# GStreamer/gst-plugins-bad

Measured on AMD Instinct MI355X. Metric: bayer2rgb Mpix/s @4K (device-resident batch), higher is better.
Workload: dtype u8

## Files before the change

gst-plugins-bad_amd/csrc/mibayer_internal.h:

```cpp
#ifndef MIBAYER_INTERNAL_H
#define MIBAYER_INTERNAL_H

#include <hip/hip_runtime.h>
#include <stddef.h>
#include <stdint.h>

namespace mibayer {

constexpr int kNumXcd = 8;

struct FastDiv {
  uint32_t d;
  uint32_t mul;
  uint32_t sh1, sh2;
};

inline FastDiv make_fastdiv (uint32_t d)
{
  FastDiv f;
  f.d = d ? d : 1;
  uint32_t l = 0;
  while (l < 32 && (1ull << l) < f.d)
    l++;
  f.mul = (uint32_t) ((((1ull << l) - f.d) << 32) / f.d + 1);
// ... 94 lines not shown
  uint32_t sel[4];
  int swap_rows;
  int nlist;
  const uint8_t *src_list[kMaxList];
  uint8_t *dst_list[kMaxList];
};

__device__ __forceinline__ const uint8_t *frame_src (const KParams &p, uint32_t frame)
{
  return p.nlist ? p.src_list[frame] : p.src + frame * p.src_frame_bytes;
}

__device__ __forceinline__ uint8_t *frame_dst (const KParams &p, uint32_t frame)
{
  return p.nlist ? p.dst_list[frame] : p.dst + frame * p.dst_frame_bytes;
}

struct Variant {
  const char *name;
  int tile_w;
  int tile_h;
  int threads;
  int band;
  int persistent;
  void (*fast) (KParams);
  void (*generic) (KParams);
  void (*aligned64) (KParams);
  void (*aligned128) (KParams);
};

int variant_count ();
const Variant &variant (int id);
int resolve_variant (int id, int width);
bool known_width_plan (int width, int *variant, int *band);
int frame_class_variant (int width, int height, int slots);
int plain_store_twin (int id);
int hybrid_store_twin (int id);
int production_shape_of (int id);

struct R2BParams {
  const uint8_t *src;
  uint8_t *dst;
  unsigned long long src_frame_bytes;
  unsigned long long dst_frame_bytes;
  int width;
  int height;
  int src_stride;
  int dst_stride;
  int out_dwords;
  long long total_rows;
  int band;
  int start_sleep;
  TileMap map;
  FastDiv div_height;
  uint32_t sel_lo[2];
  uint32_t sel_hi[2];
  int flat_k, flat_px, flat_ld, rows;
  FastDiv div_out_dwords;
  uint32_t item0, item_end;
  int nlist;
  FastDiv div_blocks_per_frame;
  const uint8_t *src_list[kMaxList];
  uint8_t *dst_list[kMaxList];
};
hipError_t launch_rgb2bayer (const R2BParams &p, bool vec16, hipStream_t stream,
    long long row0 = 0, long long nrows = -1);
hipError_t launch_rgb2bayer_list (const R2BParams &p, bool vec16, bool dst8, hipStream_t stream);

constexpr int kStripRows = 16;
struct DeepParams {
  const uint8_t *src;
  uint8_t *dst;
  unsigned long long src_frame_bytes;
  unsigned long long dst_frame_bytes;
  int width;
  int height;
  int src_stride;
  int dst_stride;
  int dn_last;
  int swap_rows;
  uint32_t in_sel;
  uint32_t mask2;
  int out_shift;
  uint32_t sel[4];
  uint32_t sel16[2][2];
  int green_odd;
  int red_odd;
  int vmax;
  uint32_t sel_cgd[2][2];
  int px3;
  int planar;
  int groups;
  FastDiv div_tiles_x;
  FastDiv div_chunks;
  uint32_t chunk0;
  uint32_t nwaves;
  int nlist;
  const uint8_t *src_list[kMaxList];
  uint8_t *dst_list[kMaxList];
};
struct ColourStage {
  int has_tone;
  int black[3];
  int m_hi[9], m_lo[9];
  uint32_t tone[257];
};
struct ColourParams {
  DeepParams d;
  int mhc;
  int in8, out16;
  ColourStage s;
};
struct StripKind { bool mhc, in8, out16; };
hipError_t launch_strip (const DeepParams &p, StripKind kind, const ColourStage *stage, int nframes, hipStream_t stream,
    long long chunk0 = 0, long long nchunks = -1);

constexpr int kHalfLanePixels = 4;
constexpr int kHalfWavePixels = 64 * kHalfLanePixels;
constexpr int kHalfGroupPixels = 4 * kHalfWavePixels;
constexpr int kHalfRows = 4;
struct HalfParams {
  DeepParams d;
  int in8, out16;
  int colour;
  ColourStage s;
};
hipError_t launch_half (const DeepParams &p, bool in8, bool out16, const ColourStage *stage, int nframes,
    hipStream_t stream);

constexpr int kStatsSegRows = 64;
constexpr int kStatsMaxZones = 64;
struct StatsParams {
  const uint8_t *src;
  unsigned long long src_frame_bytes;
  unsigned long long *stats;
  int width, height, src_stride;
  int in8;
  uint32_t in_sel;
  uint32_t mask2;
  uint32_t lo, hi;
  int zones_x, zones_y;
  int ch;
  FastDiv div_cw;
  int row_dwords;
  int segs;
  FastDiv div_strips;
};
hipError_t launch_stats (const StatsParams &p, int nframes, hipStream_t stream);

constexpr int kHistReps = 8;
constexpr int kHistAhead = 8;
constexpr int kHistMaxRows = 256;
constexpr int kHistMinRows = 16;
constexpr int kHistSpread = 512;
struct HistParams {
  const uint8_t *src;
  unsigned long long src_frame_bytes;
  uint32_t *hist;
  int src_stride;
  int in8;
  uint32_t in_sel;
  uint32_t mask2;
  int shift;
  int x0, x1, y0, y1;
  int g0, g1;
  int seg_rows;
  FastDiv div_strips;
};
hipError_t launch_hist (const HistParams &p, int nframes, hipStream_t stream);

struct FocusParams {
  const uint8_t *src;
  unsigned long long src_frame_bytes;
  unsigned long long *focus;
  int width, height, src_stride;
  int in8;
  uint32_t in_sel;
  uint32_t mask2;
  uint32_t thr;
  int zones_x, zones_y;
  int ch;
  FastDiv div_cw;
  int row_dwords;
  int segs;
  FastDiv div_strips;
};
hipError_t launch_focus (const FocusParams &p, int nframes, hipStream_t stream);

constexpr int kShadeAhead = 8;
constexpr int kShadeMaxRows = 64;
constexpr int kShadeMinRows = 16;
constexpr int kShadeSpread = 1024;
constexpr int kShadeMaxNodes = 129;
struct ShadeParams {
  const uint8_t *src;
  uint8_t *dst;
  unsigned long long src_frame_bytes, dst_frame_bytes;
  const uint16_t *table;
  int width, height, src_stride, dst_stride;
  int in8;
  uint32_t in_sel;
  uint32_t mask2;
  int vmax;
  int kx, ky;
  int nx, ny;
  int black[4];
  int y0, y1;
  int row_dwords;
  int seg_rows;
  FastDiv div_strips;
};
hipError_t launch_shade (const ShadeParams &p, int nframes, hipStream_t stream);

constexpr int kDpcMaxRows = 64;
constexpr int kDpcMinRows = 16;
constexpr int kDpcSpread = 1024;
struct DpcParams {
  const uint8_t *src;
  uint8_t *dst;
  unsigned long long src_frame_bytes, dst_frame_bytes;
  const uint32_t *list;
  int list_lo, list_hi;
  int width, height, src_stride, dst_stride;
  int in8;
  uint32_t in_sel;
  uint32_t mask2;
  int hot, cold;
  int y0, y1;
  int row_dwords;
  int seg_rows;
  FastDiv div_strips;
};
hipError_t launch_dpc (const DpcParams &p, int nframes, hipStream_t stream);

constexpr int kNrMaxRows = 64;
constexpr int kNrMinRows = 16;
constexpr int kNrSpread = 1024;
struct NrParams {
  const uint8_t *src;
  uint8_t *dst;
  unsigned long long src_frame_bytes, dst_frame_bytes;
  int width, height, src_stride, dst_stride;
  int in8;
  uint32_t in_sel;
  uint32_t mask2;
  int shift;
  int y0, y1;
  int lut[16][2];
  uint32_t rcp[26];
// ... 15 lines not shown
```

gst-plugins-bad_amd/csrc/mibayer_kernels.hip:

```cpp
#include "mibayer_internal.h"

#include <stdlib.h>
#include <type_traits>

namespace mibayer {

typedef uint32_t u32x4 __attribute__ ((ext_vector_type (4)));
typedef uint32_t u32x2 __attribute__ ((ext_vector_type (2)));
typedef uint32_t u32x4_a4 __attribute__ ((ext_vector_type (4), aligned (4)));
typedef uint32_t u32x2_a4 __attribute__ ((ext_vector_type (2), aligned (4)));
typedef uint32_t u32x3_a4 __attribute__ ((ext_vector_type (3), aligned (4)));


template <bool INTRIN>
__device__ __forceinline__ uint32_t avg4 (uint32_t a, uint32_t b)
{
  if constexpr (INTRIN) {
    return __builtin_amdgcn_lerp (a, b, 0x01010101u);
  } else {
    return (a | b) - (((a ^ b) >> 1) & 0x7f7f7f7fu);
  }
}

template <bool INTRIN>
// ... 1413 lines not shown
  }
  uint32_t q[4];
  q[0] = from_lane_below (e, hi);
  q[1] = lo;
  q[2] = hi;
  q[3] = from_lane_above (e, lo);
  if (first)
    q[0] = bsel (kLowHalves, q[2], q[1]);
  if (lastmode == 1)
    q[3] = bsel (kLowHalves, q[2], q[1]);
  if (partial)
    q[2] = bsel (kLowHalves, q[1], q[0]);
  int s[8];
#pragma unroll
  for (int i = 0; i < 4; i++) {
    s[2 * i] = (int) (q[i] & 0xffffu);
    s[2 * i + 1] = (int) (q[i] >> 16);
  }
  MhcRow r;
#pragma unroll
  for (int k = 0; k < 4; k++) {
    r.c[k] = s[k + 2];
    r.h1[k] = s[k + 1] + s[k + 3];
    r.h2[k] = s[k] + s[k + 4];
  }
  return r;
}

template <bool GREEN>
__device__ __forceinline__ void mhc_pixel (const DeepParams &p, const MhcRow &m2, const MhcRow &m1, const MhcRow &z,
    const MhcRow &p1, const MhcRow &p2, int k, int &C, int &G, int &D)
{
  const int c = z.c[k];
  const int h1 = z.h1[k], h2 = z.h2[k];
  const int v1 = m1.c[k] + p1.c[k];
  const int v2 = m2.c[k] + p2.c[k];
  const int d = m1.h1[k] + p1.h1[k];
  int f1, f2;
  if constexpr (GREEN) {
    G = c;
    f1 = 10 * c + 8 * h1 - 2 * (h2 + d) + v2;
    f2 = 10 * c + 8 * v1 - 2 * (v2 + d) + h2;
  } else {
    C = c;
    f1 = 8 * c + 4 * (h1 + v1) - 2 * (h2 + v2);
    f2 = 12 * c + 4 * d - 3 * (h2 + v2);
  }
  f1 = min (max ((f1 + 8) >> 4, 0), p.vmax);
  f2 = min (max ((f2 + 8) >> 4, 0), p.vmax);
  if constexpr (GREEN)
    C = f1;
  else
    G = f1;
  D = f2;
}

__device__ __forceinline__ int reflect_row (int r, int height)
{
  r = r < 0 ? -r : r;
  return r > height + 1 ? height - 1 : r >= height ? 2 * height - 2 - r : r;
}

template <bool OUT16>
__device__ __forceinline__ void emit_cgd (const uint32_t (&x)[4], const uint32_t (&y)[4], uint32_t s0, uint32_t s1,
    u32x4 &v0, u32x4 &v1)
{
  if constexpr (OUT16) {
    v0.x = __builtin_amdgcn_perm (x[0], y[0], s0);
    v0.y = __builtin_amdgcn_perm (x[0], y[0], s1);
    v0.z = __builtin_amdgcn_perm (x[1], y[1], s0);
    v0.w = __builtin_amdgcn_perm (x[1], y[1], s1);
    v1.x = __builtin_amdgcn_perm (x[2], y[2], s0);
    v1.y = __builtin_amdgcn_perm (x[2], y[2], s1);
    v1.z = __builtin_amdgcn_perm (x[3], y[3], s0);
    v1.w = __builtin_amdgcn_perm (x[3], y[3], s1);
  } else {
    v0.x = __builtin_amdgcn_perm (x[0], y[0], s0);
    v0.y = __builtin_amdgcn_perm (x[1], y[1], s0);
    v0.z = __builtin_amdgcn_perm (x[2], y[2], s0);
    v0.w = __builtin_amdgcn_perm (x[3], y[3], s0);
  }
}

template <bool IN8, bool OUT16>
__global__ void __launch_bounds__ (256)
bayer2rgb_mhc_kernel (DeepParams p)
{
  const uint32_t wave = (uint32_t) __builtin_amdgcn_readfirstlane ((int) (blockIdx.x * 4u + (threadIdx.x >> 6)));
  if (wave >= p.nwaves)
    return;
  const int lane = (int) (threadIdx.x & 63u);
  const uint32_t crow = fastdiv (wave, p.div_tiles_x);
  const uint32_t tx = wave - crow * p.div_tiles_x.d;
  const uint32_t chunk = p.chunk0 + crow;
  const uint32_t frame = fastdiv (chunk, p.div_chunks);
  const int y0 = (int) (chunk - frame * p.div_chunks.d) * kStripRows;
  const int y1 = y0 + kStripRows < p.height ? y0 + kStripRows : p.height;
  const uint8_t *src = p.nlist
      ? kernarg_table_entry<const uint8_t *> (offsetof (DeepParams, src_list), frame) : p.src + frame * p.src_frame_bytes;
  uint8_t *dst = p.nlist
      ? kernarg_table_entry<uint8_t *> (offsetof (DeepParams, dst_list), frame) : p.dst + frame * p.dst_frame_bytes;
  const int g = (int) tx * 64 + lane;
  const bool first = g == 0;
  const int lastmode = g == p.groups - 1 ? ((p.width & 3) ? 2 : 1) : 0;
  const bool store = g < p.groups;
  const bool full = 4 * g + 4 <= p.width;

  DeepRaw raw[kStripRows + 4];
#pragma unroll
  for (int i = 0; i < kStripRows + 4; i++)
    raw[i] = deep_load<IN8> (p, src, reflect_row (y0 - 2 + i, p.height), g, lane);
  MhcRow w0 = mhc_row<IN8> (p, raw[0], lane, first, lastmode);
  MhcRow w1 = mhc_row<IN8> (p, raw[1], lane, first, lastmode);
  MhcRow w2 = mhc_row<IN8> (p, raw[2], lane, first, lastmode);
  MhcRow w3 = mhc_row<IN8> (p, raw[3], lane, first, lastmode);
#pragma unroll
  for (int k = 0; k < kStripRows; k++) {
    const int j = y0 + k;
    if (j >= y1)
      break;
    const MhcRow w4 = mhc_row<IN8> (p, raw[k + 4], lane, first, lastmode);
    int C[4], G[4], D[4];
    if (((j & 1) ^ p.green_odd) == 0) {
      mhc_pixel<true> (p, w0, w1, w2, w3, w4, 0, C[0], G[0], D[0]);
      mhc_pixel<false> (p, w0, w1, w2, w3, w4, 1, C[1], G[1], D[1]);
      mhc_pixel<true> (p, w0, w1, w2, w3, w4, 2, C[2], G[2], D[2]);
      mhc_pixel<false> (p, w0, w1, w2, w3, w4, 3, C[3], G[3], D[3]);
    } else {
      mhc_pixel<false> (p, w0, w1, w2, w3, w4, 0, C[0], G[0], D[0]);
      mhc_pixel<true> (p, w0, w1, w2, w3, w4, 1, C[1], G[1], D[1]);
      mhc_pixel<false> (p, w0, w1, w2, w3, w4, 2, C[2], G[2], D[2]);
      mhc_pixel<true> (p, w0, w1, w2, w3, w4, 3, C[3], G[3], D[3]);
    }
    const int rk = (j & 1) ^ p.red_odd;
    const int s = p.out_shift;
    uint32_t x[4], y[4];
#pragma unroll
    for (int i = 0; i < 4; i++) {
      if constexpr (OUT16) {
        x[i] = ((uint32_t) C[i] << s) | ((uint32_t) G[i] << (16 + s));
        y[i] = (uint32_t) D[i] << s;
      } else {
        x[i] = ((uint32_t) C[i] >> s) | (((uint32_t) G[i] >> s) << 16);
        y[i] = (uint32_t) D[i] >> s;
      }
    }
    uint8_t *out = dst + (size_t) j * (size_t) p.dst_stride;
    if constexpr (OUT16) {
      const uint32_t s0 = p.sel_cgd[rk][0], s1 = p.sel_cgd[rk][1];
      u32x4 v0, v1;
      emit_cgd<true> (x, y, s0, s1, v0, v1);
      store_strip16 (p, out, g, lane, v0, v1);
    } else if (const int planes = planar_of (p)) {
      store_planes8 (p, planes, out, g, store, full, rk ? 2 : 0, rk ? 0 : 2, gather_byte<0> (x), gather_byte<2> (x),
          gather_byte<0> (y));
    } else {
      const uint32_t s0 = p.sel_cgd[rk][0];
      u32x4 v, unused;
      emit_cgd<false> (x, y, s0, s0, v, unused);
      store_strip8 (out, g, store, full, p.px3 != 0, v);
    }
    w0 = w1;
    w1 = w2;
    w2 = w3;
    w3 = w4;
  }
}


constexpr int kColourAhead = 4;

__device__ __forceinline__ DeepRaw colour_load (const ColourParams &cp, const uint8_t *src, int r, int g, int lane)
{
  const DeepParams &p = cp.d;
  if (cp.mhc) {
    r = reflect_row (r, p.height);
  } else {
    r = r < 0 ? -r : r;
    r = r == p.height ? p.dn_last : r > p.height ? p.height - 1 : r;
  }
  if (cp.in8)
    return deep_load<true> (p, src, r, g, lane);
  return deep_load<false> (p, src, r, g, lane);
}

__device__ __forceinline__ MhcRow colour_row (const ColourParams &cp, const DeepRaw &raw, int lane, bool first,
    int lastmode)
{
  MhcRow r;
  if (cp.in8)
    r = mhc_row<true> (cp.d, raw, lane, first, lastmode);
  else
    r = mhc_row<false> (cp.d, raw, lane, first, lastmode);
  if (!cp.mhc) {
// ... 549 lines not shown
        const uint32_t m = __builtin_amdgcn_perm (d, d, p.in_sel) & p.mask2;
        v[0] = m & 0xffffu;
        v[1] = m >> 16;
        v[2] = v[3] = 0;
      }
#pragma unroll
      for (int k = 0; k < 4; k++) {
        const uint32_t wk = k < 2 ? w : w & w23;
        const bool in = v[k] - p.lo <= p.hi - p.lo;
        sum[rp][k >> 1][k & 1] += in ? v[k] * wk : 0u;
        cnt[rp][k >> 1][k & 1] += in ? wk : 0u;
        clip[rp][k >> 1][k & 1] += v[k] > p.hi ? wk : 0u;
      }
    };
    int y = y0;
    for (; y + kStatsAhead <= y1; y += kStatsAhead) {
      uint32_t d[kStatsAhead];
#pragma unroll
      for (int i = 0; i < kStatsAhead; i++)
        d[i] = __builtin_nontemporal_load ((const uint32_t *) (col + (size_t) (y + i) * (size_t) p.src_stride));
#pragma unroll
      for (int i = 0; i < kStatsAhead; i++)
        add (d[i], i & 1, 1u);
    }
    for (; y < y1; y += 2) {
      const bool two = y + 1 < y1;
      const uint32_t d0 = __builtin_nontemporal_load ((const uint32_t *) (col + (size_t) y * (size_t) p.src_stride));
      const uint32_t d1 = two
          ? __builtin_nontemporal_load ((const uint32_t *) (col + (size_t) (y + 1) * (size_t) p.src_stride)) : 0u;
      add (d0, 0, 1u);
      add (d1, 1, two ? 1u : 0u);
    }
#pragma unroll
    for (int h = 0; h < 2; h++) {
      if (h == 1 && !w23)
        continue;
      const uint32_t zx = fastdiv ((uint32_t) (x0 + 2 * h), p.div_cw);
#pragma unroll
      for (int site = 0; site < 4; site++) {
        const uint32_t e = zx * 4u + (uint32_t) site;
        const uint32_t n = cnt[site >> 1][h][site & 1], c = clip[site >> 1][h][site & 1];
        if (n) {
          atomicAdd (&t_sum[e], (unsigned long long) sum[site >> 1][h][site & 1]);
          atomicAdd (&t_cnt[e], n);
        }
        if (c)
          atomicAdd (&t_clip[e], c);
      }
    }
  }
  __syncthreads ();
  const uint32_t e = threadIdx.x;
  unsigned long long *zone = p.stats
      + 8ull * (((unsigned long long) frame * (uint32_t) p.zones_y + (uint32_t) zy) * (uint32_t) p.zones_x + (e >> 2));
  if (t_cnt[e]) {
    atomicAdd (zone + (e & 3u), t_sum[e]);
    atomicAdd ((uint32_t *) (zone + 4) + (e & 3u), t_cnt[e]);
  }
  if (t_clip[e])
    atomicAdd ((uint32_t *) (zone + 6) + (e & 3u), t_clip[e]);
}

hipError_t launch_stats (const StatsParams &p, int nframes, hipStream_t stream)
{
  if (nframes <= 0)
    return nframes == 0 ? hipSuccess : hipErrorInvalidValue;
  if (p.width < 2 || (p.width & 1) || p.height < 1 || p.zones_x < 1 || p.zones_x > kStatsMaxZones || p.zones_y < 1
      || p.ch < 2 || (p.ch & 1) || p.div_cw.d < 2 || (p.div_cw.d & 1)
      || (unsigned long long) p.div_cw.d * (unsigned) p.zones_x < (unsigned) p.width
      || (long long) p.ch * p.zones_y < p.height)
    return hipErrorInvalidValue;
  StatsParams q = p;
  q.row_dwords = p.in8 ? (p.width + 3) / 4 : p.width / 2;
  q.segs = (p.ch + kStatsSegRows - 1) / kStatsSegRows;
  const long long strips = (q.row_dwords + 255) / 256;
  const long long gy = (long long) q.segs * p.zones_y;
  if (strips * nframes > 0x7fffffffLL || gy > 65535)
    return hipErrorInvalidValue;
  q.div_strips = make_fastdiv ((uint32_t) strips);
  hipLaunchKernelGGL (mosaic_stats_kernel, dim3 ((unsigned) (strips * nframes), (unsigned) gy), dim3 (256), 0, stream, q);
  return hipGetLastError ();
}

__global__ void __launch_bounds__ (256)
mosaic_hist_kernel (HistParams p)
{
  __shared__ uint32_t tab[kHistReps * 1024];
  for (int i = (int) threadIdx.x; i < kHistReps * 1024; i += 256)
    tab[i] = 0;
  __syncthreads ();
  const uint32_t frame = fastdiv (blockIdx.x, p.div_strips);
  const uint32_t strip = blockIdx.x - frame * p.div_strips.d;
  const int ya = p.y0 + (int) blockIdx.y * p.seg_rows;
  const int yb = ya + p.seg_rows < p.y1 ? ya + p.seg_rows : p.y1;
  const int g = p.g0 + (int) (strip * 256u + threadIdx.x);
  if (g < p.g1) {
    const int c0 = p.in8 ? 4 * g : 2 * g;
    const bool in0 = c0 >= p.x0 && c0 < p.x1;
    const bool in1 = p.in8 && c0 + 2 >= p.x0 && c0 + 2 < p.x1;
    const bool both = in0 && in1;
    const uint32_t swz = (threadIdx.x & (kHistReps - 1)) << 3;
    uint32_t *rep = tab + (threadIdx.x & (kHistReps - 1)) * 1024;
    const uint8_t *col = p.src + frame * p.src_frame_bytes + 4 * (size_t) g;
    for (int y = ya; y < yb; y += kHistAhead) {
      uint32_t d[kHistAhead];
#pragma unroll
      for (int i = 0; i < kHistAhead; i++)
        d[i] = y + i < yb
            ? __builtin_nontemporal_load ((const uint32_t *) (col + (size_t) (y + i) * (size_t) p.src_stride)) : 0u;
#pragma unroll
      for (int i = 0; i < kHistAhead; i++) {
        if (y + i >= yb)
          break;
        const uint32_t sb = (uint32_t) ((y + i) & 1) * 512u;
        uint32_t b0, b1, b2, b3;
        if (p.in8) {
          b0 = d[i] & 0xffu;
          b1 = (d[i] >> 8) & 0xffu;
          b2 = (d[i] >> 16) & 0xffu;
          b3 = d[i] >> 24;
        } else {
          const uint32_t m = __builtin_amdgcn_perm (d[i], d[i], p.in_sel) & p.mask2;
          b0 = b2 = (m & 0xffffu) >> p.shift;
          b1 = b3 = m >> (16 + p.shift);
        }
        const bool e02 = both && b0 == b2, e13 = both && b1 == b3;
        if (in0) {
          atomicAdd (&rep[(sb + b0) ^ swz], e02 ? 2u : 1u);
          atomicAdd (&rep[(sb + 256u + b1) ^ swz], e13 ? 2u : 1u);
        }
        if (in1 && !e02)
          atomicAdd (&rep[(sb + b2) ^ swz], 1u);
        if (in1 && !e13)
          atomicAdd (&rep[(sb + 256u + b3) ^ swz], 1u);
      }
    }
  }
  __syncthreads ();
  uint32_t *out = p.hist + (size_t) frame * 1024u;
  for (uint32_t e = threadIdx.x; e < 1024u; e += 256u) {
    uint32_t n = 0;
#pragma unroll
    for (uint32_t r = 0; r < (uint32_t) kHistReps; r++)
      n += tab[r * 1024u + (e ^ (r << 3))];
    if (n)
      atomicAdd (out + e, n);
  }
}

hipError_t launch_hist (const HistParams &p, int nframes, hipStream_t stream)
{
  if (nframes <= 0)
    return nframes == 0 ? hipSuccess : hipErrorInvalidValue;
  if (p.x0 < 0 || (p.x0 & 1) || (p.x1 & 1) || p.x1 < p.x0 + 2 || p.y0 < 0 || p.y1 < p.y0 + 1 || p.shift < 0 || p.shift > 8)
    return hipErrorInvalidValue;
  HistParams q = p;
  q.g0 = p.in8 ? p.x0 / 4 : p.x0 / 2;
  q.g1 = p.in8 ? (p.x1 + 3) / 4 : p.x1 / 2;
  const long long strips = (q.g1 - q.g0 + 255) / 256;
  const long long h = p.y1 - p.y0;
  long long rows = h * strips * nframes / kHistSpread;
  rows = rows < kHistMinRows ? kHistMinRows : rows > kHistMaxRows ? kHistMaxRows : rows;
  if ((h + rows - 1) / rows > 65535)
    rows = (h + 65534) / 65535;
  rows = (rows + 1) & ~1LL;
  const long long gy = (h + rows - 1) / rows;
  if (strips * nframes > 0x7fffffffLL || gy > 65535)
    return hipErrorInvalidValue;
  q.seg_rows = (int) rows;
  q.div_strips = make_fastdiv ((uint32_t) strips);
  hipLaunchKernelGGL (mosaic_hist_kernel, dim3 ((unsigned) (strips * nframes), (unsigned) gy), dim3 (256), 0, stream, q);
  return hipGetLastError ();
}

template <bool IN8>
__global__ void __launch_bounds__ (256)
mosaic_shade_kernel (ShadeParams p)
{
  constexpr int NS = IN8 ? 4 : 2;
  const uint32_t frame = fastdiv (blockIdx.x, p.div_strips);
  const uint32_t strip = blockIdx.x - frame * p.div_strips.d;
  const int ya = (p.y0 & ~1) + (int) blockIdx.y * p.seg_rows;
  const int yb = ya + p.seg_rows < p.y1 ? ya + p.seg_rows : p.y1;
  const int g = (int) (strip * 256u + threadIdx.x);
  if (g >= p.row_dwords)
    return;
  const int x0 = IN8 ? 4 * g : 2 * g;
  const bool tail = IN8 && x0 + 2 >= p.width;
  const bool in_place = (const uint8_t *) p.dst == p.src;
  const uint32_t cw = 1u << p.kx, ch = 1u << p.ky;
  const int sh = p.kx + p.ky;
  const uint32_t rnd = 1u << (sh - 1);
  uint32_t wl[NS], wr[NS];
#pragma unroll
  for (int k = 0; k < NS; k++) {
    wr[k] = (uint32_t) (x0 + k) & (cw - 1u);
    wl[k] = cw - wr[k];
  }
  const uint16_t *tab = p.table + (x0 >> p.kx);
  auto node_row = [&] (int jr, uint32_t (&h)[2][NS]) {
#pragma unroll
    for (int s = 0; s < 4; s++) {
      const uint16_t *n = tab + ((size_t) s * (size_t) p.ny + (size_t) jr) * (size_t) p.nx;
      const uint32_t l = n[0], r = n[1];
#pragma unroll
      for (int k = s & 1; k < NS; k += 2)
        h[s >> 1][k] = l * wl[k] + r * wr[k];
    }
  };
  const uint8_t *scol = p.src + frame * p.src_frame_bytes + 4 * (size_t) g;
  uint8_t *dcol = p.dst + frame * p.dst_frame_bytes + 4 * (size_t) g;
  int j = ya >> p.ky;
  uint32_t a[2][NS], b[2][NS];
  node_row (j, a);
  node_row (j + 1, b);
  for (int y = ya; y < yb;) {
    if ((y >> p.ky) != j) {
      j = y >> p.ky;
#pragma unroll
      for (int k = 0; k < NS; k++) {
        a[0][k] = b[0][k];
        a[1][k] = b[1][k];
      }
      node_row (j + 1, b);
    }
    const int seam = (j + 1) << p.ky;
    const int ye = seam < yb ? seam : yb;
    for (int yy = y; yy < ye; yy += kShadeAhead) {
      const uint32_t fy0 = (uint32_t) yy & (ch - 1u);
      uint32_t d[kShadeAhead];
#pragma unroll
      for (int i = 0; i < kShadeAhead; i++)
        d[i] = yy + i < ye
            ? __builtin_nontemporal_load ((const uint32_t *) (scol + (size_t) (yy + i) * (size_t) p.src_stride)) : 0u;
#pragma unroll
      for (int i = 0; i < kShadeAhead; i++) {
        if (yy + i >= ye)
          break;
        if (yy + i < p.y0)
          continue;
        const uint32_t fy = fy0 + (uint32_t) i;
        uint32_t v[NS];
        if (IN8) {
#pragma unroll
          for (int k = 0; k < NS; k++)
            v[k] = (d[i] >> (8 * k)) & 0xffu;
        } else {
          const uint32_t m = __builtin_amdgcn_perm (d[i], d[i], p.in_sel) & p.mask2;
          v[0] = m & 0xffffu;
          v[NS - 1] = m >> 16;
        }
        uint32_t o = 0;
#pragma unroll
        for (int k = 0; k < NS; k++) {
// ... 664 lines not shown
```

gst-plugins-bad_amd/csrc/mibayer_abi.hip:

```cpp
#include "../../include/mibayer.h"
#include "mibayer_hooks.h"
#include "mibayer_internal.h"

#include <dlfcn.h>
#include <sys/syscall.h>
#include <unistd.h>

#include <algorithm>
#include <atomic>
#include <limits.h>
#include <math.h>
#include <memory>
#include <mutex>
#include <new>
#include <stdio.h>
#include <stdlib.h>
#include <string.h>
#include <time.h>
#include <vector>

using namespace mibayer;

#ifdef MIBAYER_LAB
#define LAB_GETENV(name) getenv (name)
// ... 602 lines not shown
static void plan_selectors (const mibayer_cfg &f, uint32_t sel[4],
    int &swap_rows)
{
  int rp = f.r_off, bp = f.b_off, gp = f.g_off;
  if (f.pattern == MIBAYER_RGGB || f.pattern == MIBAYER_GBRG) {
    int t = rp;
    rp = bp;
    bp = t;
  }
  swap_rows = (f.pattern == MIBAYER_GRBG || f.pattern == MIBAYER_GBRG);
  const int ap = 6 - rp - gp - bp;
  for (int k = 0; k < 4; k++) {
    uint32_t s = 0;
    s |= (uint32_t) (4 + 2 * (k & 1)) << (8 * rp);
    s |= (uint32_t) (5 + 2 * (k & 1)) << (8 * bp);
    s |= (uint32_t) k << (8 * gp);
    s |= (uint32_t) 0x0d << (8 * ap);
    sel[k] = s;
  }
}

struct SampleFormat {
  int bits;
  bool in8;
  uint32_t in_sel;
  uint32_t vmax;
  uint32_t mask2;
};

static SampleFormat sample_format (const mibayer_cfg &f)
{
  SampleFormat sf;
  const int bits = (int) ((f.flags & MIBAYER_FLAG_SRC_BITS_MASK) >> 8);
  sf.bits = bits ? bits : 8;
  sf.in8 = bits == 0;
  sf.in_sel = (f.flags & MIBAYER_FLAG_SRC_BIG_ENDIAN) ? 0x02030001u : 0x03020100u;
  sf.vmax = (1u << sf.bits) - 1u;
  sf.mask2 = sf.vmax * 0x00010001u;
  return sf;
}

static void make_plan (mibayer_ctx *c)
{
  plan_selectors (c->cfg, c->sel, c->swap_rows);
}

static void make_cgd_selectors (mibayer_ctx *c, int depth)
{
  const mibayer_cfg &f = c->cfg;
  DeepParams &q = c->deep_args;
  q.green_odd = f.pattern == MIBAYER_BGGR || f.pattern == MIBAYER_RGGB;
  q.red_odd = f.pattern == MIBAYER_BGGR || f.pattern == MIBAYER_GBRG;
  q.vmax = (1 << depth) - 1;
  const bool be = (f.flags & MIBAYER_FLAG_DST_BIG_ENDIAN) != 0;
  for (int rk = 0; rk < 2; rk++) {
    const int r_lo = rk == 0 ? 4 : 0, b_lo = rk == 0 ? 0 : 4;
    if (!c->kind.out16) {
      uint32_t s = 0;
      for (int ch = 0; ch < 4; ch++) {
        const uint32_t b = ch == f.r_off ? r_lo : ch == f.b_off ? b_lo : ch == f.g_off ? 6 : 0x0d;
        s |= b << (8 * ch);
      }
      q.sel_cgd[rk][0] = q.sel_cgd[rk][1] = s;
      continue;
    }
    for (int d = 0; d < 2; d++) {
      uint32_t s = 0;
      for (int slot = 0; slot < 2; slot++) {
        const int ch = 2 * d + slot;
        uint32_t lo = ch == f.r_off ? r_lo : ch == f.b_off ? b_lo : ch == f.g_off ? 6 : 0x0d;
        uint32_t hi = lo == 0x0d ? 0x0d : lo + 1;
        if (be) {
          const uint32_t t = lo;
          lo = hi;
          hi = t;
        }
        s |= (lo << (16 * slot)) | (hi << (16 * slot + 8));
      }
      q.sel_cgd[rk][d] = s;
    }
  }
}

static void make_deep_plan (mibayer_ctx *c)
{
  const mibayer_cfg &f = c->cfg;
  const SampleFormat sf = sample_format (f);
  const int depth = sf.bits;
  c->kind.in8 = sf.in8;
  c->kind.out16 = (f.flags & MIBAYER_FLAG_DST_16BIT) != 0;
  DeepParams &q = c->deep_args;
  q = DeepParams ();
  q.width = c->half ? c->out_width : f.width;
  q.height = c->half ? c->out_height : f.height;
  q.src_stride = f.src_stride;
  q.dst_stride = f.dst_stride;
  q.dn_last = f.height >= 4 ? f.height - 4 : 1;
  q.swap_rows = c->swap_rows;
  q.in_sel = sf.in_sel;
  q.mask2 = sf.mask2;
  q.out_shift = c->kind.out16 ? 16 - depth : depth - 8;
  q.px3 = (f.flags & MIBAYER_FLAG_DST_24BIT) != 0;
  if (f.flags & MIBAYER_FLAG_DST_PLANAR) {
    const bool swap = !(c->kind.mhc || c->colour || c->half) && (f.pattern == MIBAYER_RGGB || f.pattern == MIBAYER_GBRG);
    q.planar = 0x100 | (swap ? f.b_off : f.r_off) | f.g_off << 2 | (swap ? f.r_off : f.b_off) << 4;
  }
  if (c->kind.mhc || c->colour || c->half)
    make_cgd_selectors (c, depth);
  for (int k = 0; k < 4; k++)
    q.sel[k] = c->sel[k];
  int rp = f.r_off, bp = f.b_off;
  if (f.pattern == MIBAYER_RGGB || f.pattern == MIBAYER_GBRG) {
    rp = f.b_off;
    bp = f.r_off;
  }
  const bool be = (f.flags & MIBAYER_FLAG_DST_BIG_ENDIAN) != 0;
  for (int h = 0; h < 2; h++)
    for (int d = 0; d < 2; d++) {
      uint32_t s = 0;
      for (int slot = 0; slot < 2; slot++) {
        const int ch = 2 * d + slot;
        uint32_t lo, hi;
        if (ch == rp) {
          lo = 4;
          hi = 5;
        } else if (ch == bp) {
          lo = 6;
          hi = 7;
        } else if (ch == f.g_off) {
          lo = (uint32_t) (2 * h);
          hi = lo + 1;
        } else {
          lo = hi = 0x0d;
        }
        if (be) {
          const uint32_t t = lo;
          lo = hi;
          hi = t;
        }
        s |= (lo << (16 * slot)) | (hi << (16 * slot + 8));
      }
      q.sel16[h][d] = s;
    }
}

static void colour_snapshot (const mibayer_ctx *c, ColourStage *st)
{
  std::lock_guard<std::mutex> lk (c->colour_mu);
  *st = c->colour_stage;
}

static int launch_deep_kernel (const mibayer_ctx *c, DeepParams &q, int nframes, hipStream_t stream,
    long long chunk0 = 0, long long nchunks = -1, const ColourStage *stage = nullptr)
{
  ColourStage now;
  if (!c->colour) {
    stage = nullptr;
  } else if (!stage) {
    colour_snapshot (c, &now);
    stage = &now;
  }
  if (c->half) {
    if (chunk0 != 0 || nchunks >= 0)
      return MIBAYER_ERR_ARG;
    HIP_TRY (launch_half (q, c->kind.in8, c->kind.out16, stage, nframes, stream));
    return MIBAYER_OK;
  }
  HIP_TRY (launch_strip (q, c->kind, stage, nframes, stream, chunk0, nchunks));
  return MIBAYER_OK;
}

struct FrameSet {
  const uint8_t *src;
  uint8_t *dst;
  size_t src_frame_bytes, dst_frame_bytes;
  const void *const *srcs;
  void *const *dsts;
  int n;

  static FrameSet strided (const void *src, size_t src_frame_bytes, void *dst, size_t dst_frame_bytes, int nframes)
  {
    return { (const uint8_t *) src, (uint8_t *) dst, src_frame_bytes, dst_frame_bytes, nullptr, nullptr, nframes };
  }
  static FrameSet list (const void *const *srcs, void *const *dsts, int n)
  {
    return { nullptr, nullptr, 0, 0, srcs, dsts, n };
  }
  bool is_list () const { return srcs != nullptr; }
  template <typename T>
  bool on_grid (T *const *list, const void *base, size_t frame_bytes, unsigned a) const
  {
    if (!list)
      return (((uintptr_t) base) & (a - 1)) == 0 && (n == 1 || frame_bytes % a == 0);
    for (int f = 0; f < n; f++)
      if (((uintptr_t) list[f]) & (a - 1))
        return false;
    return true;
  }
  bool srcs16 () const { return on_grid (srcs, src, src_frame_bytes, 16); }
  bool all16 () const { return srcs16 () && on_grid (dsts, dst, dst_frame_bytes, 16); }
  bool dsts8 () const { return on_grid (dsts, dst, dst_frame_bytes, 8); }
  bool dst_on_grid (unsigned a) const { return !is_list () && on_grid (dsts, dst, dst_frame_bytes, a); }
  template <typename P>
  void fill (P &p) const
  {
    p.src = src;
    p.dst = dst;
    p.src_frame_bytes = src_frame_bytes;
    p.dst_frame_bytes = dst_frame_bytes;
    p.nlist = is_list () ? n : 0;
    for (int f = 0; f < p.nlist; f++) {
      p.src_list[f] = (const uint8_t *) srcs[f];
      p.dst_list[f] = (uint8_t *) dsts[f];
    }
  }
};

static FrameSet slot_frame (const mibayer_ctx *c, const Slot &s)
{
  return FrameSet::strided (s.d_src, c->src_bytes, s.d_dst, c->dst_bytes, 1);
}

constexpr int kFrameClassRounds = 4;

static int launch_class (const mibayer_ctx *c, long long nframes)
{
// ... 3410 lines not shown
```

Before: 1.307 million.

## Restructure histogram kernel with packed 16-bit LDS counters and 16-byte loads

Rewrites the mosaic histogram kernel. The block grows to 512 threads split into two row groups, and each lane loads 16 bytes when alignment allows. Counts go into a per-lane-column LDS table that packs two 16-bit counters per word instead of eight swizzled replicas. Rows from all frames are flattened into chunks that can span frame boundaries, and each chunk is merged to global memory after it is processed. The aim is less LDS atomic contention, fewer load instructions and better load balance across frames, at the cost of more frequent syncs and merges and a tighter counter overflow bound.

```diff
diff --git a/gst-plugins-bad_amd/csrc/mibayer_internal.h b/gst-plugins-bad_amd/csrc/mibayer_internal.h
--- a/gst-plugins-bad_amd/csrc/mibayer_internal.h
+++ b/gst-plugins-bad_amd/csrc/mibayer_internal.h
@@ -266,11 +266,22 @@
 };
 hipError_t launch_stats (const StatsParams &p, int nframes, hipStream_t stream);
 
-constexpr int kHistReps = 8;
-constexpr int kHistAhead = 8;
-constexpr int kHistMaxRows = 256;
+constexpr int kHistWaves = 4;
+constexpr int kHistRowGroups = 2;
+constexpr int kHistThreads = 64 * kHistWaves * kHistRowGroups;
+constexpr int kHistLaneBytes = 16;
+constexpr int kHistCols = 32;
+constexpr int kHistRowWords = 256 * kHistCols;
+constexpr int kHistFieldPerRow = (kHistLaneBytes / 2) * (64 / kHistCols) * kHistWaves;
+constexpr int kHistFieldRows = 2 * (65535 / kHistFieldPerRow);
+constexpr int kHistAhead = 4;
+constexpr int kHistMaxRows = 512;
 constexpr int kHistMinRows = 16;
 constexpr int kHistSpread = 512;
+static_assert (kHistMaxRows <= kHistFieldRows && kHistFieldPerRow * ((kHistFieldRows + 1) / 2) <= 65535,
+    "a 16-bit counter field of the histogram table could overflow before the merge");
+static_assert (64 % kHistCols == 0 && kHistCols % 4 == 0 && kHistMaxRows % 2 == 0 && kHistMinRows % 2 == 0
+    && kHistThreads == 2 * 256, "");
 struct HistParams {
   const uint8_t *src;
   unsigned long long src_frame_bytes;
@@ -281,8 +292,11 @@
   uint32_t mask2;
   int shift;
   int x0, x1, y0, y1;
+  int wide;
   int g0, g1;
   int seg_rows;
+  uint32_t total_rows;
+  FastDiv div_h;
   FastDiv div_strips;
 };
 hipError_t launch_hist (const HistParams &p, int nframes, hipStream_t stream);
diff --git a/gst-plugins-bad_amd/csrc/mibayer_kernels.hip b/gst-plugins-bad_amd/csrc/mibayer_kernels.hip
--- a/gst-plugins-bad_amd/csrc/mibayer_kernels.hip
+++ b/gst-plugins-bad_amd/csrc/mibayer_kernels.hip
@@ -2262,69 +2262,116 @@
   return hipGetLastError ();
 }
 
-__global__ void __launch_bounds__ (256)
+__device__ __forceinline__ void hist_count (const HistParams &p, uint32_t *row_tab, uint32_t d, bool in0, bool in1)
+{
+  uint32_t b0, b1, b2, b3;
+  if (p.in8) {
+    b0 = d & 0xffu;
+    b1 = (d >> 8) & 0xffu;
+    b2 = (d >> 16) & 0xffu;
+    b3 = d >> 24;
+  } else {
+    const uint32_t m = __builtin_amdgcn_perm (d, d, p.in_sel) & p.mask2;
+    b0 = b2 = (m & 0xffffu) >> p.shift;
+    b1 = b3 = m >> (16 + p.shift);
+  }
+  const bool both = in0 && in1;
+  const bool e02 = both && b0 == b2, e13 = both && b1 == b3;
+  if (in0) {
+    atomicAdd (&row_tab[b0 * kHistCols], e02 ? 2u : 1u);
+    atomicAdd (&row_tab[b1 * kHistCols], e13 ? 0x20000u : 0x10000u);
+  }
+  if (in1 && !e02)
+    atomicAdd (&row_tab[b2 * kHistCols], 1u);
+  if (in1 && !e13)
+    atomicAdd (&row_tab[b3 * kHistCols], 0x10000u);
+}
+
+template <int N, int A>
+__device__ __forceinline__ void hist_walk (const HistParams &p, uint32_t *lane_tab, const uint8_t *col, int g, int ya, int yb)
+{
+  typedef typename std::conditional<N == 4, u32x4, uint32_t>::type T;
+  bool in0[N], in1[N];
+#pragma unroll
+  for (int k = 0; k < N; k++) {
+    const int c0 = p.in8 ? 4 * (g + k) : 2 * (g + k);
+    in0[k] = c0 >= p.x0 && c0 < p.x1;
+    in1[k] = p.in8 && c0 + 2 >= p.x0 && c0 + 2 < p.x1;
+  }
+  constexpr int S = A * kHistRowGroups;
+  T cur[A], nxt[A];
+#pragma unroll
+  for (int i = 0; i < A; i++)
+    cur[i] = ya + i < yb ? __builtin_nontemporal_load ((const T *) (col + (size_t) (ya + i) * (size_t) p.src_stride)) : T (0);
+  for (int y = ya; y < yb; y += S) {
+#pragma unroll
+    for (int i = 0; i < A; i++)
+      nxt[i] = y + S + i < yb
+          ? __builtin_nontemporal_load ((const T *) (col + (size_t) (y + S + i) * (size_t) p.src_stride)) : T (0);
+#pragma unroll
+    for (int i = 0; i < A; i++) {
+      if (y + i < yb) {
+        uint32_t *row_tab = lane_tab + ((y + i) & 1) * kHistRowWords;
+        if constexpr (N == 4) {
+#pragma unroll
+          for (int k = 0; k < N; k++)
+            hist_count (p, row_tab, cur[i][k], in0[k], in1[k]);
+        } else
+          hist_count (p, row_tab, cur[i], in0[0], in1[0]);
+      }
+      cur[i] = nxt[i];
+    }
+  }
+}
+
+__global__ void __launch_bounds__ (kHistThreads)
 mosaic_hist_kernel (HistParams p)
 {
-  __shared__ uint32_t tab[kHistReps * 1024];
-  for (int i = (int) threadIdx.x; i < kHistReps * 1024; i += 256)
-    tab[i] = 0;
+  __shared__ u32x4 tab4[2 * kHistRowWords / 4];
+  uint32_t *tab = (uint32_t *) tab4;
+  for (int i = (int) threadIdx.x; i < 2 * kHistRowWords / 4; i += kHistThreads)
+    tab4[i] = u32x4 (0);
   __syncthreads ();
-  const uint32_t frame = fastdiv (blockIdx.x, p.div_strips);
-  const uint32_t strip = blockIdx.x - frame * p.div_strips.d;
-  const int ya = p.y0 + (int) blockIdx.y * p.seg_rows;
-  const int yb = ya + p.seg_rows < p.y1 ? ya + p.seg_rows : p.y1;
-  const int g = p.g0 + (int) (strip * 256u + threadIdx.x);
-  if (g < p.g1) {
-    const int c0 = p.in8 ? 4 * g : 2 * g;
-    const bool in0 = c0 >= p.x0 && c0 < p.x1;
-    const bool in1 = p.in8 && c0 + 2 >= p.x0 && c0 + 2 < p.x1;
-    const bool both = in0 && in1;
-    const uint32_t swz = (threadIdx.x & (kHistReps - 1)) << 3;
-    uint32_t *rep = tab + (threadIdx.x & (kHistReps - 1)) * 1024;
-    const uint8_t *col = p.src + frame * p.src_frame_bytes + 4 * (size_t) g;
-    for (int y = ya; y < yb; y += kHistAhead) {
-      uint32_t d[kHistAhead];
-#pragma unroll
-      for (int i = 0; i < kHistAhead; i++)
-        d[i] = y + i < yb
-            ? __builtin_nontemporal_load ((const uint32_t *) (col + (size_t) (y + i) * (size_t) p.src_stride)) : 0u;
-#pragma unroll
-      for (int i = 0; i < kHistAhead; i++) {
-        if (y + i >= yb)
-          break;
-        const uint32_t sb = (uint32_t) ((y + i) & 1) * 512u;
-        uint32_t b0, b1, b2, b3;
-        if (p.in8) {
-          b0 = d[i] & 0xffu;
-          b1 = (d[i] >> 8) & 0xffu;
-          b2 = (d[i] >> 16) & 0xffu;
-          b3 = d[i] >> 24;
-        } else {
-          const uint32_t m = __builtin_amdgcn_perm (d[i], d[i], p.in_sel) & p.mask2;
-          b0 = b2 = (m & 0xffffu) >> p.shift;
-          b1 = b3 = m >> (16 + p.shift);
-        }
-        const bool e02 = both && b0 == b2, e13 = both && b1 == b3;
-        if (in0) {
-          atomicAdd (&rep[(sb + b0) ^ swz], e02 ? 2u : 1u);
-          atomicAdd (&rep[(sb + 256u + b1) ^ swz], e13 ? 2u : 1u);
-        }
-        if (in1 && !e02)
-          atomicAdd (&rep[(sb + b2) ^ swz], 1u);
-        if (in1 && !e13)
-          atomicAdd (&rep[(sb + 256u + b3) ^ swz], 1u);
+  const uint32_t chunk = fastdiv (blockIdx.x, p.div_strips);
+  const uint32_t strip = blockIdx.x - chunk * p.div_strips.d;
+  const int lane = (int) threadIdx.x & (64 * kHistWaves - 1);
+  const int group = (int) threadIdx.x / (64 * kHistWaves);
+  const int g = p.g0 + ((int) strip * 64 * kHistWaves + lane) * (p.wide ? 4 : 1);
+  uint32_t row = chunk * (uint32_t) p.seg_rows;
+  const uint32_t end = row + (uint32_t) p.seg_rows < p.total_rows ? row + (uint32_t) p.seg_rows : p.total_rows;
+  while (row < end) {
+    const uint32_t frame = fastdiv (row, p.div_h);
+    const int ya = p.y0 + (int) (row - frame * p.div_h.d);
+    const int yb = (uint32_t) (p.y1 - ya) < end - row ? p.y1 : ya + (int) (end - row);
+    if (g < p.g1) {
+      const uint8_t *col = p.src + frame * p.src_frame_bytes + 4 * (size_t) g;
+      uint32_t *lane_tab = tab + (threadIdx.x & (kHistCols - 1));
+      if (p.wide)
+        hist_walk<4, kHistAhead> (p, lane_tab, col, g, ya + group * kHistAhead, yb);
+      else
+        hist_walk<1, 2 * kHistAhead> (p, lane_tab, col, g, ya + group * 2 * kHistAhead, yb);
+    }
+    __syncthreads ();
+    uint32_t n0 = 0, n1 = 0;
+    u32x4 *own = tab4 + threadIdx.x * (kHistCols / 4);
+#pragma unroll
+    for (uint32_t k = 0; k < (uint32_t) kHistCols / 4; k++) {
+      const uint32_t s = ((threadIdx.x >> 1) + k) & (kHistCols / 4 - 1);
+      const u32x4 w = own[s];
+      own[s] = u32x4 (0);
+#pragma unroll
+      for (int j = 0; j < 4; j++) {
+        n0 += w[j] & 0xffffu;
+        n1 += w[j] >> 16;
       }
     }
-  }
-  __syncthreads ();
-  uint32_t *out = p.hist + (size_t) frame * 1024u;
-  for (uint32_t e = threadIdx.x; e < 1024u; e += 256u) {
-    uint32_t n = 0;
-#pragma unroll
-    for (uint32_t r = 0; r < (uint32_t) kHistReps; r++)
-      n += tab[r * 1024u + (e ^ (r << 3))];
-    if (n)
-      atomicAdd (out + e, n);
+    uint32_t *out = p.hist + (size_t) frame * 1024u + (threadIdx.x >> 8) * 512u + (threadIdx.x & 255u);
+    if (n0)
+      atomicAdd (out, n0);
+    if (n1)
+      atomicAdd (out + 256, n1);
+    __syncthreads ();
+    row += (uint32_t) (yb - ya);
   }
 }
 
@@ -2335,21 +2382,29 @@
   if (p.x0 < 0 || (p.x0 & 1) || (p.x1 & 1) || p.x1 < p.x0 + 2 || p.y0 < 0 || p.y1 < p.y0 + 1 || p.shift < 0 || p.shift > 8)
     return hipErrorInvalidValue;
   HistParams q = p;
+  q.wide = ((uintptr_t) p.src | (uintptr_t) p.src_stride | (nframes > 1 ? p.src_frame_bytes : 0)) % kHistLaneBytes == 0;
   q.g0 = p.in8 ? p.x0 / 4 : p.x0 / 2;
+  if (q.wide)
+    q.g0 &= ~(kHistLaneBytes / 4 - 1);
   q.g1 = p.in8 ? (p.x1 + 3) / 4 : p.x1 / 2;
-  const long long strips = (q.g1 - q.g0 + 255) / 256;
-  const long long h = p.y1 - p.y0;
-  long long rows = h * strips * nframes / kHistSpread;
+  const long long lane_dwords = q.wide ? kHistLaneBytes / 4 : 1;
+  const long long strips = (q.g1 - q.g0 + 64 * kHistWaves * lane_dwords - 1) / (64 * kHistWaves * lane_dwords);
+  const long long h = p.y1 - p.y0, total = h * nframes;
+  if (total > 0x7fffffffLL)
+    return hipErrorInvalidValue;
+  const long long per_round = (long long) kHistSpread * kHistMaxRows;
+  const long long rounds = (total * strips + per_round - 1) / per_round;
+  long long rows = total * strips / (kHistSpread * rounds);
   rows = rows < kHistMinRows ? kHistMinRows : rows > kHistMaxRows ? kHistMaxRows : rows;
-  if ((h + rows - 1) / rows > 65535)
-    rows = (h + 65534) / 65535;
   rows = (rows + 1) & ~1LL;
-  const long long gy = (h + rows - 1) / rows;
-  if (strips * nframes > 0x7fffffffLL || gy > 65535)
+  const long long chunks = (total + rows - 1) / rows;
+  if (strips * chunks > 0x7fffffffLL)
     return hipErrorInvalidValue;
   q.seg_rows = (int) rows;
+  q.total_rows = (uint32_t) total;
+  q.div_h = make_fastdiv ((uint32_t) h);
   q.div_strips = make_fastdiv ((uint32_t) strips);
-  hipLaunchKernelGGL (mosaic_hist_kernel, dim3 ((unsigned) (strips * nframes), (unsigned) gy), dim3 (256), 0, stream, q);
+  hipLaunchKernelGGL (mosaic_hist_kernel, dim3 ((unsigned) (strips * chunks)), dim3 (kHistThreads), 0, stream, q);
   return hipGetLastError ();
 }
 
```

After: 1.293 million. 0.989x the previous value.

## Add packed 16-bit SIMD path for 8-bit MHC demosaic

Applied to the files above, without the earlier changes.

For 8-bit input with 8-bit output, the Malvar-He-Cutler kernel now computes two pixels per lane at a time using packed 16-bit vector arithmetic (s16x2), with byte-permute selectors for neighbour gathering and output interleaving. The weights are forced into scalar registers and the rounding clamps with packed min and max. This aims to roughly halve the ALU instruction count per pixel in a kernel that may be compute-bound. In exchange it adds a separate code path, plus a union of the old selectors with new packed selectors that is only valid when colour, half and 16-bit modes are off.

```diff
diff --git a/gst-plugins-bad_amd/csrc/mibayer_abi.hip b/gst-plugins-bad_amd/csrc/mibayer_abi.hip
--- a/gst-plugins-bad_amd/csrc/mibayer_abi.hip
+++ b/gst-plugins-bad_amd/csrc/mibayer_abi.hip
@@ -708,6 +708,21 @@
   }
 }
 
+static void make_packed_selectors (mibayer_ctx *c)
+{
+  const mibayer_cfg &f = c->cfg;
+  DeepParams &q = c->deep_args;
+  for (int rk = 0; rk < 2; rk++)
+    for (int half = 0; half < 2; half++) {
+      const uint32_t C = 4 + 2 * half, G = 5 + 2 * half, D = 2 * half;
+      const uint32_t R = rk == 0 ? C : D, B = rk == 0 ? D : C;
+      uint32_t s = 0;
+      for (int ch = 0; ch < 4; ch++)
+        s |= (ch == f.r_off ? R : ch == f.b_off ? B : ch == f.g_off ? G : 0x0du) << (8 * ch);
+      q.sel_pk[rk][half] = s;
+    }
+}
+
 static void make_deep_plan (mibayer_ctx *c)
 {
   const mibayer_cfg &f = c->cfg;
@@ -768,6 +783,8 @@
       }
       q.sel16[h][d] = s;
     }
+  if (c->kind.mhc && c->kind.in8 && !c->kind.out16 && !c->colour && !c->half)
+    make_packed_selectors (c);
 }
 
 static void colour_snapshot (const mibayer_ctx *c, ColourStage *st)
diff --git a/gst-plugins-bad_amd/csrc/mibayer_internal.h b/gst-plugins-bad_amd/csrc/mibayer_internal.h
--- a/gst-plugins-bad_amd/csrc/mibayer_internal.h
+++ b/gst-plugins-bad_amd/csrc/mibayer_internal.h
@@ -200,7 +200,10 @@
   uint32_t in_sel;
   uint32_t mask2;
   int out_shift;
-  uint32_t sel[4];
+  union {
+    uint32_t sel[4];
+    uint32_t sel_pk[2][2];
+  };
   uint32_t sel16[2][2];
   int green_odd;
   int red_odd;
diff --git a/gst-plugins-bad_amd/csrc/mibayer_kernels.hip b/gst-plugins-bad_amd/csrc/mibayer_kernels.hip
--- a/gst-plugins-bad_amd/csrc/mibayer_kernels.hip
+++ b/gst-plugins-bad_amd/csrc/mibayer_kernels.hip
@@ -1519,6 +1519,135 @@
   }
 }
 
+typedef short s16x2 __attribute__ ((ext_vector_type (2)));
+
+template <bool IN8, bool OUT16> constexpr bool kMhcPacked = IN8 && !OUT16;
+
+struct MhcPkSel { uint32_t el, ol, er, orr; bool tail; };
+struct MhcPkRow { s16x2 e, o, h1e, h1o, h2e, h2o; };
+
+__device__ __forceinline__ MhcPkSel mhc_pk_sel (bool first, int lastmode)
+{
+  MhcPkSel s;
+  s.el = first ? 0x0c000c02u : 0x0c000c06u;
+  s.ol = first ? 0x0c010c01u : 0x0c010c07u;
+  s.er = 0x0c040c02u;
+  s.orr = 0x0c050c03u;
+  if (lastmode == 1) {
+    s.er = 0x0c020c02u;
+    s.orr = 0x0c010c03u;
+  }
+  if (lastmode == 2) {
+    s.er = 0x0c040c00u;
+    s.orr = 0x0c050c07u;
+  }
+  s.tail = lastmode == 2;
+  return s;
+}
+
+__device__ __forceinline__ s16x2 as_s16x2 (uint32_t v) { return __builtin_bit_cast (s16x2, v); }
+__device__ __forceinline__ uint32_t as_u32 (s16x2 v) { return __builtin_bit_cast (uint32_t, v); }
+
+__device__ __forceinline__ MhcPkRow mhc_pk_row (const DeepRaw &raw, const MhcPkSel &s)
+{
+  const uint32_t a = raw.a;
+  const uint32_t l = from_lane_below (raw.e, a);
+  uint32_t r = from_lane_above (raw.e, a);
+  r = s.tail ? l : r;
+  MhcPkRow w;
+  w.e = as_s16x2 (__builtin_amdgcn_perm (a, a, 0x0c020c00u));
+  w.o = as_s16x2 (__builtin_amdgcn_perm (a, a, 0x0c030c01u));
+  const s16x2 el = as_s16x2 (__builtin_amdgcn_perm (l, a, s.el)), ol = as_s16x2 (__builtin_amdgcn_perm (l, a, s.ol));
+  const s16x2 er = as_s16x2 (__builtin_amdgcn_perm (r, a, s.er)), orr = as_s16x2 (__builtin_amdgcn_perm (r, a, s.orr));
+  w.h1e = ol + w.o;
+  w.h1o = w.e + er;
+  w.h2e = el + er;
+  w.h2o = ol + orr;
+  return w;
+}
+
+__device__ __forceinline__ uint32_t mhc_pk_round (s16x2 acc)
+{
+  const s16x2 zero = { 0, 0 }, top = { 255, 255 };
+  return as_u32 (__builtin_elementwise_min (__builtin_elementwise_max (acc >> 4, zero), top));
+}
+
+struct MhcPkWeights { s16x2 k8, k4, km2; };
+
+__device__ __forceinline__ s16x2 mhc_pk_weight (uint32_t twice)
+{
+  asm ("" : "+s" (twice));
+  return as_s16x2 (twice);
+}
+
+__device__ __forceinline__ void mhc_pk_green (const MhcPkWeights &k, s16x2 c, s16x2 h1, s16x2 h2, s16x2 v1, s16x2 v2,
+    s16x2 d, uint32_t &C, uint32_t &D)
+{
+  const s16x2 t = c * (short) 10 + k.k8;
+  C = mhc_pk_round ((h2 + d) * k.km2 + (h1 * k.k8 + t) + v2);
+  D = mhc_pk_round ((v2 + d) * k.km2 + (v1 * k.k8 + t) + h2);
+}
+
+__device__ __forceinline__ void mhc_pk_other (const MhcPkWeights &k, s16x2 c, s16x2 h1, s16x2 h2, s16x2 v1, s16x2 v2,
+    s16x2 d, uint32_t &G, uint32_t &D)
+{
+  const s16x2 s = h2 + v2;
+  G = mhc_pk_round (s * k.km2 + ((h1 + v1) * k.k4 + (c * k.k8 + k.k8)));
+  D = mhc_pk_round (s * (short) -3 + (d * k.k4 + (c * (short) 12 + k.k8)));
+}
+
+__device__ __forceinline__ void mhc_packed_strip (const DeepParams &p, const DeepRaw (&raw)[kStripRows + 4], uint8_t *dst,
+    int y0, int y1, int g, bool first, int lastmode, bool store, bool full)
+{
+  const MhcPkSel sel = mhc_pk_sel (first, lastmode);
+  const MhcPkWeights wt = { mhc_pk_weight (0x00080008u), mhc_pk_weight (0x00040004u), mhc_pk_weight (0xfffefffeu) };
+  MhcPkRow w0 = mhc_pk_row (raw[0], sel);
+  MhcPkRow w1 = mhc_pk_row (raw[1], sel);
+  MhcPkRow w2 = mhc_pk_row (raw[2], sel);
+  MhcPkRow w3 = mhc_pk_row (raw[3], sel);
+#pragma unroll
+  for (int k = 0; k < kStripRows; k++) {
+    const int j = y0 + k;
+    if (j >= y1)
+      break;
+    const MhcPkRow w4 = mhc_pk_row (raw[k + 4], sel);
+    const s16x2 v1e = w1.e + w3.e, v1o = w1.o + w3.o;
+    const s16x2 v2e = w0.e + w4.e, v2o = w0.o + w4.o;
+    const s16x2 de = w1.h1e + w3.h1e, dod = w1.h1o + w3.h1o;
+    uint32_t ce, ge, dde, co, go, ddo;
+    if (((j & 1) ^ p.green_odd) == 0) {
+      ge = as_u32 (w2.e);
+      mhc_pk_green (wt, w2.e, w2.h1e, w2.h2e, v1e, v2e, de, ce, dde);
+      co = as_u32 (w2.o);
+      mhc_pk_other (wt, w2.o, w2.h1o, w2.h2o, v1o, v2o, dod, go, ddo);
+    } else {
+      ce = as_u32 (w2.e);
+      mhc_pk_other (wt, w2.e, w2.h1e, w2.h2e, v1e, v2e, de, ge, dde);
+      go = as_u32 (w2.o);
+      mhc_pk_green (wt, w2.o, w2.h1o, w2.h2o, v1o, v2o, dod, co, ddo);
+    }
+    const int rk = (j & 1) ^ p.red_odd;
+    uint8_t *out = dst + (size_t) j * (size_t) p.dst_stride;
+    if (const int planes = planar_of (p)) {
+      store_planes8 (p, planes, out, g, store, full, rk ? 2 : 0, rk ? 0 : 2, __builtin_amdgcn_perm (co, ce, 0x06020400u),
+          __builtin_amdgcn_perm (go, ge, 0x06020400u), __builtin_amdgcn_perm (ddo, dde, 0x06020400u));
+    } else {
+      const uint32_t cge = ce | (ge << 8), cgo = co | (go << 8);
+      const uint32_t s0 = p.sel_pk[rk][0], s1 = p.sel_pk[rk][1];
+      u32x4 v;
+      v.x = __builtin_amdgcn_perm (cge, dde, s0);
+      v.y = __builtin_amdgcn_perm (cgo, ddo, s0);
+      v.z = __builtin_amdgcn_perm (cge, dde, s1);
+      v.w = __builtin_amdgcn_perm (cgo, ddo, s1);
+      store_strip8 (out, g, store, full, p.px3 != 0, v);
+    }
+    w0 = w1;
+    w1 = w2;
+    w2 = w3;
+    w3 = w4;
+  }
+}
+
 template <bool IN8, bool OUT16>
 __global__ void __launch_bounds__ (256)
 bayer2rgb_mhc_kernel (DeepParams p)
@@ -1547,6 +1676,10 @@
 #pragma unroll
   for (int i = 0; i < kStripRows + 4; i++)
     raw[i] = deep_load<IN8> (p, src, reflect_row (y0 - 2 + i, p.height), g, lane);
+  if constexpr (kMhcPacked<IN8, OUT16>) {
+    mhc_packed_strip (p, raw, dst, y0, y1, g, first, lastmode, store, full);
+    return;
+  }
   MhcRow w0 = mhc_row<IN8> (p, raw[0], lane, first, lastmode);
   MhcRow w1 = mhc_row<IN8> (p, raw[1], lane, first, lastmode);
   MhcRow w2 = mhc_row<IN8> (p, raw[2], lane, first, lastmode);
```

Result: no change. 1.287 million before, 1.286 million after (-0.1%).
